# Qervas/cn_chess_ai

Hardware: AMD Instinct MI355X
Metric: env steps/sec + DQN updates/sec at 8192 parallel games, 1/2/4/8 MI355X (higher is better)
Workload: dtype f32

## Files before the change

cn_chess_ai_amd/csrc/xq_rules.hip.h:

```cpp
#pragma once

#include "xq_common.h"

namespace xq {

struct __attribute__((aligned(16))) WaveSlab {
    float q[96];
    uint16_t moves[kMaxMoves];
    uint8_t sq[96];
    int32_t misc[8];
};

__device__ __forceinline__ int lane_id() { return (int)(threadIdx.x & 63u); }

__device__ __forceinline__ int at(const uint8_t* sq, int r, int c) {
    return ((unsigned)r < 10u && (unsigned)c < 9u) ? (int)sq[r * 9 + c] : 0;
}
__device__ __forceinline__ bool inside(int r, int c) { return (unsigned)r < 10u && (unsigned)c < 9u; }
__device__ __forceinline__ bool in_any_palace(int r, int c) {
    return c >= 3 && c <= 5 && ((r >= 0 && r <= 2) || (r >= 7 && r <= 9));
}
__device__ __forceinline__ bool in_own_palace(int color, int r, int c) {
    return c >= 3 && c <= 5 && (color == C_RED ? (r >= 0 && r <= 2) : (r >= 7 && r <= 9));
}
__device__ __forceinline__ bool same_side(int a, int b) { return (a > 7) == (b > 7); }

__device__ __forceinline__ int count_between(const uint8_t* sq, int fr, int fc, int tr, int tc) {
    int n = 0;
    if (fr == tr) {
        const int step = tc > fc ? 1 : -1;
        for (int c = fc + step; c != tc; c += step) n += at(sq, fr, c) != 0;
    } else {
        const int step = tr > fr ? 1 : -1;
        for (int r = fr + step; r != tr; r += step) n += at(sq, r, fc) != 0;
    }
    return n;
}

__device__ inline bool piece_rule(const uint8_t* sq, int type, int fr, int fc, int tr, int tc) {
    const int dr = tr - fr, dc = tc - fc;
    const int adr = dr < 0 ? -dr : dr, adc = dc < 0 ? -dc : dc;
    switch (type) {
        case T_GENERAL:
            return in_any_palace(fr, fc) && in_any_palace(tr, tc) && adr + adc == 1;
        case T_ADVISOR:
            return in_any_palace(tr, tc) && adr == 1 && adc == 1;
        case T_ELEPHANT:
            return adr == 2 && adc == 2 && ((fr < 5 && tr < 5) || (fr >= 5 && tr >= 5)) && at(sq, (fr + tr) / 2, (fc + tc) / 2) == 0;
        case T_HORSE:
            return ((adr == 2 && adc == 1) || (adr == 1 && adc == 2)) && at(sq, fr + dr / 2, fc + dc / 2) == 0;
        case T_CHARIOT:
            return (fr == tr || fc == tc) && count_between(sq, fr, fc, tr, tc) == 0;
        case T_CANNON: {
            if (fr != tr && fc != tc) return false;
            const int n = count_between(sq, fr, fc, tr, tc);
            return at(sq, tr, tc) == 0 ? n == 0 : n == 1;
        }
        case T_SOLDIER: {
            const int f = at(sq, fr, fc);
            if (f >= 1 && f <= 7) return fr < 5 ? (dr == 1 && adc == 0) : ((dr == 1 && adc == 0) || (dr == 0 && adc == 1));
            return fr >= 5 ? (dr == -1 && adc == 0) : ((dr == -1 && adc == 0) || (dr == 0 && adc == 1));
        }
        default: return false;
    }
}

__device__ inline bool is_valid_move(const uint8_t* sq, int fr, int fc, int tr, int tc) {
    if (!inside(fr, fc) || !inside(tr, tc)) return false;
    const int f = sq[fr * 9 + fc], t = sq[tr * 9 + tc];
    if (f == 0) return false;
    if (t != 0 && same_side(f, t)) return false;
    return piece_rule(sq, code_type(f), fr, fc, tr, tc);
}

template <int CTRL, int ROW_MASK>
__device__ __forceinline__ int dpp_int(int identity, int v) {
    return __builtin_amdgcn_update_dpp(identity, v, CTRL, ROW_MASK, 0xf, false);
}
__device__ __forceinline__ int wave_inclusive_scan(int v) {
    v += dpp_int<0x111, 0xf>(0, v);
    v += dpp_int<0x112, 0xf>(0, v);
    v += dpp_int<0x114, 0xf>(0, v);
    v += dpp_int<0x118, 0xf>(0, v);
    v += dpp_int<0x142, 0xa>(0, v);
    v += dpp_int<0x143, 0xc>(0, v);
    return v;
}
__device__ __forceinline__ int wave_sum(int v) {
    return __builtin_amdgcn_readlane(wave_inclusive_scan(v), 63);
}
__device__ __forceinline__ void wave_sync() {
    __builtin_amdgcn_fence(__ATOMIC_RELEASE, "wavefront");
    __builtin_amdgcn_wave_barrier();
    __builtin_amdgcn_fence(__ATOMIC_ACQUIRE, "wavefront");
}
__device__ __forceinline__ float wave_max(float v) {
    const int ninf = __float_as_int(-__builtin_inff());
    auto step = [&](int t) { v = fmaxf(v, __int_as_float(t)); };
    step(dpp_int<0x111, 0xf>(ninf, __float_as_int(v)));
    step(dpp_int<0x112, 0xf>(ninf, __float_as_int(v)));
    step(dpp_int<0x114, 0xf>(ninf, __float_as_int(v)));
    step(dpp_int<0x118, 0xf>(ninf, __float_as_int(v)));
    step(dpp_int<0x142, 0xa>(ninf, __float_as_int(v)));
    step(dpp_int<0x143, 0xc>(ninf, __float_as_int(v)));
    return __int_as_float(__builtin_amdgcn_readlane(__float_as_int(v), 63));
}

__device__ __forceinline__ void unpack_to_slab(uint32_t word, uint8_t* sq) {
    const int lane = lane_id();
    if (lane < kBoardWords) {
        const uint32_t lo = word & 0xFFFFu, hi = word >> 16;
        auto spread = [](uint32_t x) -> uint32_t {
            return (x & 0xFu) | ((x & 0xF0u) << 4) | ((x & 0xF00u) << 8) | ((x & 0xF000u) << 12);
        };
        reinterpret_cast<uint32_t*>(sq)[lane * 2] = spread(lo);
        reinterpret_cast<uint32_t*>(sq)[lane * 2 + 1] = spread(hi);
    }
}
__device__ __forceinline__ uint32_t pack_from_slab(const uint8_t* sq) {
    const int lane = lane_id();
    uint32_t v = 0;
    if (lane < kBoardWords) {
        const uint32_t a = reinterpret_cast<const uint32_t*>(sq)[lane * 2];
        const uint32_t b = reinterpret_cast<const uint32_t*>(sq)[lane * 2 + 1];
        auto squeeze = [](uint32_t x) -> uint32_t {
            return (x & 0xFu) | ((x >> 4) & 0xF0u) | ((x >> 8) & 0xF00u) | ((x >> 12) & 0xF000u);
        };
        v = squeeze(a) | (squeeze(b) << 16);
    }
    return v;
}

struct Mask90 { unsigned long long lo, hi; };
__device__ __forceinline__ unsigned bits_at(const Mask90& m, int pos, unsigned mask) {
    const unsigned long long a = (m.lo >> (pos & 63)) | ((m.hi << 1) << (63 - (pos & 63)));
    const unsigned long long b = m.hi >> (pos & 63);
    return (unsigned)(pos >= 64 ? b : a) & mask;
}

struct RayHit { int empties, first, second; };
__device__ __forceinline__ RayHit ray_scan(unsigned line, int pos, int len, bool forward) {
    const unsigned l = forward ? line : (__brev(line) >> (32 - len));
    const int p = forward ? pos : len - 1 - pos;
    const unsigned x = l >> (p + 1);
    const int e = __ffs((int)x) - 1;
    const unsigned y = x >> ((e + 1) & 31);
    const int e2 = __ffs((int)y) - 1;
    int first = x ? p + 1 + e : -1;
    int second = (x && y) ? p + 2 + e + e2 : -1;
    RayHit h;
    h.empties = x ? e : len - 1 - p;
    h.first = (first >= 0 && !forward) ? len - 1 - first : first;
    h.second = (second >= 0 && !forward) ? len - 1 - second : second;
    return h;
}

__device__ inline int gen_all_actions(WaveSlab& slab, int player) {
    const int lane = lane_id();
    const uint8_t* sq = slab.sq;
    const int p0 = sq[lane];
    const int p1 = lane < 26 ? sq[64 + lane] : 0;
    const bool black = player == C_BLACK;
    Mask90 occ, own, occT;
    occ.lo = __ballot(p0 != 0); occ.hi = __ballot(p1 != 0);
    const bool o0 = p0 != 0 && (p0 > 7) == black, o1 = p1 != 0 && (p1 > 7) == black;
    own.lo = __ballot(o0); own.hi = __ballot(o1);
    {
        const int t0 = lane, t1 = 64 + lane;
        const int s0 = (t0 % 10) * 9 + t0 / 10;
        const int s1 = t1 < 90 ? (t1 % 10) * 9 + t1 / 10 : 0;
        occT.lo = __ballot(sq[s0] != 0);
        occT.hi = __ballot(t1 < 90 && sq[s1] != 0);
    }
    uint8_t* rank_sq = reinterpret_cast<uint8_t*>(slab.misc);
    const unsigned long long below = (1ull << lane) - 1ull;
    const int n_lo = __popcll(own.lo);
    const int n_own = n_lo + __popcll(own.hi);
    if (o0) { const int k = __popcll(own.lo & below); if (k < 16) rank_sq[k] = (uint8_t)lane; }
    if (o1) { const int k = n_lo + __popcll(own.hi & below); if (k < 16) rank_sq[k] = (uint8_t)(64 + lane); }
    wave_sync();

    int total = 0;
#pragma unroll 1
    for (int pass = 0; pass < 2; ++pass) {
        if (pass * 8 >= n_own) break;
        const int k = pass * 8 + (lane >> 3), slot = lane & 7;
        const bool active = k < n_own;
        const int from = rank_sq[active ? k : 0];
        const int p = sq[from];
        const int row = (from * 57) >> 9, col = from - row * 9;
        const int type = p > 7 ? p - 7 : p;
        const bool isG = type == T_GENERAL, isA = type == T_ADVISOR, isE = type == T_ELEPHANT, isH = type == T_HORSE;
        const bool isS = type == T_SOLDIER, isRay = type == T_CHARIOT || type == T_CANNON;
        const bool lt4 = slot < 4, lt2 = slot < 2;
        const int sg1 = (slot & 1) ? -1 : 1, sg2 = (slot & 2) ? -1 : 1;
        const int fw = black ? -1 : 1;
        const bool crossed = black ? row < 5 : row > 4;
        const int mag = isE ? 2 : 1;
        int dr = lt2 ? mag : -mag, dc = sg1 * mag;
        if (isG) { dr = lt2 ? sg1 : 0; dc = lt2 ? 0 : sg1; }
        if (isH) { dr = lt4 ? sg2 : 2 * sg2; dc = lt4 ? 2 * sg1 : sg1; }
        if (isS) { dr = slot == 0 ? fw : 0; dc = slot == 1 ? -1 : (slot == 2 ? 1 : 0); }
        const bool slot_ok = isH || (isS ? (slot == 0 || (slot < 3 && crossed)) : ((isG || isA || isE) && lt4));
        const int nr = row + dr, nc = col + dc;
        const bool in = inside(nr, nc);
        const bool to_pal_col = nc >= 3 && nc <= 5;
        const bool to_any_pal = to_pal_col && (nr <= 2 || nr >= 7);
        const bool to_own_pal = to_pal_col && (black ? nr >= 7 : nr <= 2);
        const bool rule = isG ? (in_any_palace(row, col) && to_any_pal)
                        : isA ? to_own_pal
                        : isE ? ((black ? nr >= 5 : nr <= 4) && ((row < 5) == (nr < 5)))
                        : true;
        bool ok = active && slot_ok && in && rule;
        const int gsq = (ok && (isE || isH)) ? (row + dr / 2) * 9 + col + dc / 2 : -1;
        const int tsq = ok ? nr * 9 + nc : from;
        const int gp = sq[gsq >= 0 ? gsq : from], tp = sq[tsq];
        ok = ok && (gsq < 0 || gp == 0) && (tp == 0 || (tp > 7) != black);
        int n_run = ok ? 1 : 0, t0 = tsq, delta = 0, extra = -1;
        if (active && isRay && lt4) {
            const bool horiz = lt2, fwd = (slot & 1) == 0;
            const unsigned line = horiz ? bits_at(occ, row * 9, 0x1FFu) : bits_at(occT, col * 10, 0x3FFu);
            const int pos = horiz ? col : row, len = horiz ? 9 : 10;
            const RayHit h = ray_scan(line, pos, len, fwd);
            delta = horiz ? (fwd ? 1 : -1) : (fwd ? 9 : -9);
            t0 = from + delta;
            n_run = h.empties;
            const int hit = type == T_CHARIOT ? h.first : h.second;
            if (hit >= 0) {
                const int bs = horiz ? row * 9 + hit : hit * 9 + col;
                if ((sq[bs] > 7) != black) {
                    if (type == T_CHARIOT) n_run += 1;
                    else extra = bs;
                }
            }
        }
        const int cnt = n_run + (extra >= 0 ? 1 : 0);
        const int inc = wave_inclusive_scan(cnt);
        const int off = total + inc - cnt;
        const int room = kMaxMoves - off;
        const int n_put = n_run < room ? n_run : (room > 0 ? room : 0);
        uint16_t* dst = slab.moves + off;
        int code = from * 90 + t0;
#pragma clang loop unroll(disable)
        for (int i = 0; i < n_put; ++i, code += delta) dst[i] = (uint16_t)code;
        if (extra >= 0 && n_run < room) dst[n_run] = (uint16_t)(from * 90 + extra);
        total += __builtin_amdgcn_readlane(inc, 63);
    }
    return total < kMaxMoves ? total : kMaxMoves;
}

__device__ __forceinline__ int piece_value(int code) {
    const int t = code_type(code);
    return t == T_GENERAL ? 1000 : t == T_ADVISOR ? 20 : t == T_ELEPHANT ? 20 : t == T_HORSE ? 40
         : t == T_CHARIOT ? 90 : t == T_CANNON ? 45 : t == T_SOLDIER ? 10 : 0;
}

__device__ inline int evaluate_board_wave(const uint8_t* sq, int color, int move_count) {
    const int lane = lane_id();
    const int p0 = sq[lane];
    const int p1 = lane < 26 ? sq[64 + lane] : 0;
    int v = 0;
    if (p0) v += ((p0 > 7) == (color == C_BLACK)) ? piece_value(p0) : -piece_value(p0);
    if (p1) v += ((p1 > 7) == (color == C_BLACK)) ? piece_value(p1) : -piece_value(p1);
    const int score = wave_sum(v);
    {
#pragma clang fp contract(off)
        const double pen = __dmul_rn((double)move_count, 0.1);
        const double x = __dsub_rn((double)score, pen);
        return (int)x;
    }
}

struct BoardStatus {
    bool red_general, black_general;
    int first_general_color;
};
__device__ inline BoardStatus board_status_wave(const uint8_t* sq) {
    const int lane = lane_id();
    const int p0 = sq[lane];
    const int p1 = lane < 26 ? sq[64 + lane] : 0;
    const unsigned long long ra = __ballot(p0 == 1), rb = __ballot(p1 == 1);
    const unsigned long long ba = __ballot(p0 == 8), bb = __ballot(p1 == 8);
    BoardStatus st;
    st.red_general = (ra | rb) != 0;
    st.black_general = (ba | bb) != 0;
    const unsigned long long ga = ra | ba, gb = rb | bb;
    if (ga) st.first_general_color = ((ra >> (__ffsll((long long)ga) - 1)) & 1ull) ? C_RED : C_BLACK;
    else if (gb) st.first_general_color = ((rb >> (__ffsll((long long)gb) - 1)) & 1ull) ? C_RED : C_BLACK;
    else st.first_general_color = C_NONE;
    return st;
}

}
```

Baseline: 47.75 million.

## Compact move-gen lanes to live piece/direction slots via prefix-sum mapping

Replaces the fixed 8-lanes-per-piece mapping over two passes with a compacted mapping. Each piece gets only as many lanes as it has possible directions (horse 8, soldier 1 or 3, others 4), assigned through a DPP prefix scan and a marks bitmap in the moves buffer. The goal is to cut idle lanes so move generation usually finishes in one wave pass instead of two. It adds a scan, ballots, shared-memory writes and an early return when there are no pieces. It also reuses the moves buffer as scratch space, which only works if nothing reads that buffer before it is written.

```diff
diff --git a/cn_chess_ai_amd/csrc/xq_rules.hip.h b/cn_chess_ai_amd/csrc/xq_rules.hip.h
--- a/cn_chess_ai_amd/csrc/xq_rules.hip.h
+++ b/cn_chess_ai_amd/csrc/xq_rules.hip.h
@@ -173,20 +173,51 @@
         occT.hi = __ballot(t1 < 90 && sq[s1] != 0);
     }
     uint8_t* rank_sq = reinterpret_cast<uint8_t*>(slab.misc);
+    uint8_t* first_slot = rank_sq + 16;
+    uint8_t* marks = reinterpret_cast<uint8_t*>(slab.moves);
     const unsigned long long below = (1ull << lane) - 1ull;
     const int n_lo = __popcll(own.lo);
     const int n_own = n_lo + __popcll(own.hi);
+    if (n_own == 0) return 0;
+    if (lane < 32) reinterpret_cast<uint32_t*>(marks)[lane] = 0u;
     if (o0) { const int k = __popcll(own.lo & below); if (k < 16) rank_sq[k] = (uint8_t)lane; }
     if (o1) { const int k = n_lo + __popcll(own.hi & below); if (k < 16) rank_sq[k] = (uint8_t)(64 + lane); }
     wave_sync();
 
+    const int n_use = n_own < 16 ? n_own : 16;
+    int live = 0;
+    if (lane < n_use) {
+        const int f = rank_sq[lane];
+        const int pc = sq[f];
+        const int t = pc > 7 ? pc - 7 : pc;
+        const int r = (f * 57) >> 9;
+        live = t == T_HORSE ? 8 : (t == T_SOLDIER ? ((black ? r < 5 : r > 4) ? 3 : 1) : 4);
+    }
+    int live_incl = live;
+    live_incl += dpp_int<0x111, 0xf>(0, live_incl);
+    live_incl += dpp_int<0x112, 0xf>(0, live_incl);
+    live_incl += dpp_int<0x114, 0xf>(0, live_incl);
+    live_incl += dpp_int<0x118, 0xf>(0, live_incl);
+    const int n_live = __builtin_amdgcn_readlane(live_incl, 15);
+    if (lane < n_use) {
+        first_slot[lane] = (uint8_t)(live_incl - live);
+        marks[live_incl - live] = 1;
+    }
+    wave_sync();
+    const int mark_lo = marks[lane], mark_hi = marks[64 + lane];
+    const unsigned long long m_lo = __ballot(mark_lo != 0), m_hi = __ballot(mark_hi != 0);
+    wave_sync();
+
     int total = 0;
 #pragma unroll 1
-    for (int pass = 0; pass < 2; ++pass) {
-        if (pass * 8 >= n_own) break;
-        const int k = pass * 8 + (lane >> 3), slot = lane & 7;
-        const bool active = k < n_own;
-        const int from = rank_sq[active ? k : 0];
+    for (int base = 0; base < n_live; base += 64) {
+        const unsigned long long mm = base ? m_hi : m_lo;
+        const int mine = base ? mark_hi : mark_lo;
+        const int k = (base ? __popcll(m_lo) : 0) + (mine != 0 ? 0 : -1)
+                    + (int)__builtin_amdgcn_mbcnt_hi((unsigned)(mm >> 32), __builtin_amdgcn_mbcnt_lo((unsigned)mm, 0u));
+        const bool active = base + lane < n_live;
+        const int from = rank_sq[k];
+        const int slot = base + lane - (int)first_slot[k];
         const int p = sq[from];
         const int row = (from * 57) >> 9, col = from - row * 9;
         const int type = p > 7 ? p - 7 : p;
@@ -195,13 +226,11 @@
         const bool lt4 = slot < 4, lt2 = slot < 2;
         const int sg1 = (slot & 1) ? -1 : 1, sg2 = (slot & 2) ? -1 : 1;
         const int fw = black ? -1 : 1;
-        const bool crossed = black ? row < 5 : row > 4;
         const int mag = isE ? 2 : 1;
         int dr = lt2 ? mag : -mag, dc = sg1 * mag;
         if (isG) { dr = lt2 ? sg1 : 0; dc = lt2 ? 0 : sg1; }
         if (isH) { dr = lt4 ? sg2 : 2 * sg2; dc = lt4 ? 2 * sg1 : sg1; }
         if (isS) { dr = slot == 0 ? fw : 0; dc = slot == 1 ? -1 : (slot == 2 ? 1 : 0); }
-        const bool slot_ok = isH || (isS ? (slot == 0 || (slot < 3 && crossed)) : ((isG || isA || isE) && lt4));
         const int nr = row + dr, nc = col + dc;
         const bool in = inside(nr, nc);
         const bool to_pal_col = nc >= 3 && nc <= 5;
@@ -211,13 +240,13 @@
                         : isA ? to_own_pal
                         : isE ? ((black ? nr >= 5 : nr <= 4) && ((row < 5) == (nr < 5)))
                         : true;
-        bool ok = active && slot_ok && in && rule;
+        bool ok = active && in && rule;
         const int gsq = (ok && (isE || isH)) ? (row + dr / 2) * 9 + col + dc / 2 : -1;
         const int tsq = ok ? nr * 9 + nc : from;
         const int gp = sq[gsq >= 0 ? gsq : from], tp = sq[tsq];
         ok = ok && (gsq < 0 || gp == 0) && (tp == 0 || (tp > 7) != black);
         int n_run = ok ? 1 : 0, t0 = tsq, delta = 0, extra = -1;
-        if (active && isRay && lt4) {
+        if (active && isRay) {
             const bool horiz = lt2, fwd = (slot & 1) == 0;
             const unsigned line = horiz ? bits_at(occ, row * 9, 0x1FFu) : bits_at(occT, col * 10, 0x3FFu);
             const int pos = horiz ? col : row, len = horiz ? 9 : 10;
```

New measurement: 47.32 million, median of 2. About the same (-0.9%).
